# joshuacwnewton/swiftwatcher

Hardware: AMD Instinct MI355X
Metric: frames/sec (segment+classify) on 1080p ROI batches (higher is better)
Workload: dtype f64 (image_filtering), f32 (CNN)

## Files before the change

### swiftwatcher_amd/csrc/cnn_common.h

```cpp
#pragma once
#include "swk_internal.h"

#include <cstring>

namespace swk {

typedef float f16v __attribute__((ext_vector_type(16)));
typedef __bf16 bf16x8 __attribute__((ext_vector_type(8)));

struct Place {
    float *dst;
    int dH, dW, dC, off_y, off_x, c_off;
};
struct Crop {
    int sh, sw, crop_y, crop_x;
};

inline bool place_ok(const Place &p, int h, int w, int c, bool quads, const Crop *crop = nullptr)
{
    if (!p.dst || c < 1 || p.off_y < 0 || p.off_x < 0 || p.off_y + h > p.dH || p.off_x + w > p.dW || p.c_off < 0 || p.c_off + c > p.dC) return false;
    if (quads && ((c & 3) || (p.dC & 3) || (p.c_off & 3) || ((uintptr_t)p.dst & 15))) return false;
    return !crop || (crop->crop_y >= 0 && crop->crop_x >= 0 && crop->crop_y + h <= crop->sh && crop->crop_x + w <= crop->sw);
}

int launch_expand1x1_split_bf16(hipStream_t s, const float *src, int64_t rows, const Crop &cr, int cin, int h, int w, const float *wgt,
                                const float *bias, int cout, const Place &pl);
extern int g_expand_split_bf16;

__device__ __forceinline__ void store_bias_relu(float *q, const f16v &acc, int g, const float4 b)
{
    float4 v;
    v.x = fmaxf(acc[4 * g] + b.x, 0.0f);
    v.y = fmaxf(acc[4 * g + 1] + b.y, 0.0f);
    v.z = fmaxf(acc[4 * g + 2] + b.z, 0.0f);
    v.w = fmaxf(acc[4 * g + 3] + b.w, 0.0f);
    *(float4 *)q = v;
}

__device__ __forceinline__ void split3(float x, __bf16 &a, __bf16 &b, __bf16 &c)
{
    a = (__bf16)x;
    const float r = x - (float)a;
    b = (__bf16)r;
    c = (__bf16)(r - (float)b);
}
inline void split3_host(float x, uint16_t part[3])
{
    for (int i = 0; i < 3; ++i) {
        uint32_t u;
        float back;
        memcpy(&u, &x, 4);
        u = (u + 0x7fffu + ((u >> 16) & 1u)) & 0xffff0000u;
        memcpy(&back, &u, 4);
        part[i] = (uint16_t)(u >> 16);
        x -= back;
    }
}

inline void winograd_U(const float g[9], double U[4][4])
{
    static const double G[4][3] = {{1.0, 0.0, 0.0}, {0.5, 0.5, 0.5}, {0.5, -0.5, 0.5}, {0.0, 0.0, 1.0}};
    double tmp[4][3];
    for (int a = 0; a < 4; ++a)
        for (int c = 0; c < 3; ++c) tmp[a][c] = G[a][0] * g[c] + G[a][1] * g[3 + c] + G[a][2] * g[6 + c];
    for (int a = 0; a < 4; ++a)
        for (int c = 0; c < 4; ++c) U[a][c] = tmp[a][0] * G[c][0] + tmp[a][1] * G[c][1] + tmp[a][2] * G[c][2];
}

template <int N>
__device__ __forceinline__ void lds_dma_copy(unsigned lds, const void *g, unsigned voff)
{
    static_assert(N >= 1 && N <= 3, "1 KB pieces per statement");
    unsigned keep;
#define SWK_LDS_DMA(pieces)                                                                                                 \
    asm volatile("s_mov_b32 %0, m0\n\ts_mov_b32 m0, %2\n\ts_nop 0\n\t" pieces "s_mov_b32 m0, %0" : "=&s"(keep) : "v"(voff), "s"(lds), "s"(g) : "memory")
#define SWK_LDS_DMA_PIECE(offset) "global_load_lds_dwordx4 %1, %3" offset "\n\t"
    if constexpr (N == 1) SWK_LDS_DMA(SWK_LDS_DMA_PIECE(""));
    else if constexpr (N == 2) SWK_LDS_DMA(SWK_LDS_DMA_PIECE("") SWK_LDS_DMA_PIECE(" offset:1024"));
    else SWK_LDS_DMA(SWK_LDS_DMA_PIECE("") SWK_LDS_DMA_PIECE(" offset:1024") SWK_LDS_DMA_PIECE(" offset:2048"));
#undef SWK_LDS_DMA_PIECE
#undef SWK_LDS_DMA
}
template <int KEEP>
__device__ __forceinline__ void lds_dma_wait()
{
    asm volatile("s_waitcnt vmcnt(%0)" ::"n"(KEEP) : "memory");
}

}
```

### swiftwatcher_amd/csrc/cnn_conv1x1.hip

```cpp
#include "cnn_common.h"

namespace swk {

template <int NBLK, int KC, int D, int CS, int NWV>
__global__ __launch_bounds__(64 * NWV) void k_conv1x1_relu_place(const float *__restrict__ src, int64_t rows, int sh, int sw, int cin, int crop_y,
                                                            int crop_x, int h, int w, const float *__restrict__ wgt, const float *__restrict__ bias,
                                                            int cout, float *__restrict__ dst, int dH, int dW, int dC, int off_y, int off_x, int c_off,
                                                            FastDiv fhw, FastDiv fw)
{
    constexpr int NP = 32 * NBLK, PITCH = NP + 1, KH = KC / 2, NV = KH / 4, NB = NBLK / CS, NT = 64 * NWV, SLOTS = NWV / CS;
    static_assert(NBLK % CS == 0 && NWV % CS == 0, "column splits");
    extern __shared__ float lds[];
    const int tid = threadIdx.x, lane = tid & 63, wave = tid >> 6, r = lane & 31, hh = lane >> 5;
    float *lbias = lds + ((cin * PITCH + 3) & ~3);
    const int hw = h * w;
    const int cs = wave % CS;
    const int64_t ntiles = (rows + 31) >> 5, stride = (int64_t)gridDim.x * SLOTS;
    int64_t tile = (int64_t)blockIdx.x * SLOTS + wave / CS;

    auto locate = [&](int64_t t, int64_t &ro) -> const float * {
        const unsigned m = (unsigned)t * 32u + (unsigned)r;
        const bool valid = m < (unsigned)rows;
        const unsigned mm = valid ? m : (unsigned)rows - 1u;
        const unsigned b = fhw.div(mm), rem = mm - b * (unsigned)hw;
        const unsigned y = fw.div(rem), x = rem - y * (unsigned)w;
        ro = valid ? (((int64_t)b * dH + off_y + y) * dW + off_x + x) * (int64_t)dC + c_off + 32 * NB * cs : -1;
        return src + (((int64_t)b * sh + crop_y + y) * sw + crop_x + x) * (int64_t)cin + KH * hh;
    };
    float4 a[D][NV];
    int64_t ro = -1, ro_next = -1;
    const float *p = src, *pn = src;
    if (tile < ntiles) {
        p = locate(tile, ro);
#pragma unroll
        for (int d = 0; d < D; ++d)
#pragma unroll
            for (int v = 0; v < NV; ++v) a[d][v] = *(const float4 *)(p + KC * d + 4 * v);
    }
    for (int co = tid >> 4; co < NP; co += NT / 16)
        for (int c4 = (tid & 15) * 4; c4 < cin; c4 += 64) {
            const float4 wv = co < cout ? *(const float4 *)(wgt + (int64_t)co * cin + c4) : make_float4(0.0f, 0.0f, 0.0f, 0.0f);
            float *q = lds + c4 * PITCH + co;
            q[0] = wv.x; q[PITCH] = wv.y; q[2 * PITCH] = wv.z; q[3 * PITCH] = wv.w;
        }
    for (int i = tid; i < NP; i += NT) lbias[i] = i < cout ? bias[i] : 0.0f;
    __syncthreads();

    for (; tile < ntiles; tile += stride) {
        const bool more = tile + stride < ntiles;
        if (more) pn = locate(tile + stride, ro_next);
        f16v acc[NB];
#pragma unroll
        for (int nb = 0; nb < NB; ++nb)
#pragma unroll
            for (int e = 0; e < 16; ++e) acc[nb][e] = 0.0f;
        for (int kb = 0; kb < cin; kb += KC * D) {
#pragma unroll
            for (int d = 0; d < D; ++d) {
                const int k0 = kb + KC * d;
                float av[KH];
#pragma unroll
                for (int v = 0; v < NV; ++v) { av[4 * v] = a[d][v].x; av[4 * v + 1] = a[d][v].y; av[4 * v + 2] = a[d][v].z; av[4 * v + 3] = a[d][v].w; }
                const int kn = k0 + KC * D;
                if (kn < cin) {
#pragma unroll
                    for (int v = 0; v < NV; ++v) a[d][v] = *(const float4 *)(p + kn + 4 * v);
                } else if (more) {
#pragma unroll
                    for (int v = 0; v < NV; ++v) a[d][v] = *(const float4 *)(pn + kn - cin + 4 * v);
                }
                const float *wrow = lds + (k0 + KH * hh) * PITCH + 32 * NB * cs + r;
                float bw[2][NB];
#pragma unroll
                for (int nb = 0; nb < NB; ++nb) bw[0][nb] = wrow[32 * nb];
#pragma unroll
                for (int i = 0; i < KH; ++i) {
                    if (i < KH - 1) {
#pragma unroll
                        for (int nb = 0; nb < NB; ++nb) bw[(i + 1) & 1][nb] = wrow[(i + 1) * PITCH + 32 * nb];
                    }
#pragma unroll
                    for (int nb = 0; nb < NB; ++nb) acc[nb] = __builtin_amdgcn_mfma_f32_32x32x2f32(bw[i & 1][nb], av[i], acc[nb], 0, 0, 0);
                    if (i < KH - 1) __builtin_amdgcn_sched_group_barrier(0x100 , NB, 0);
                    __builtin_amdgcn_sched_group_barrier(0x008 , NB, 0);
                }
            }
        }
        if (ro >= 0) {
            float *o = dst + ro + 4 * hh;
#pragma unroll
            for (int nb = 0; nb < NB; ++nb)
#pragma unroll
                for (int g = 0; g < 4; ++g) {
                    const int c = nb * 32 + 8 * g;
                    if (32 * NB * cs + c + 4 * hh < cout) store_bias_relu(o + c, acc[nb], g, *(const float4 *)(lbias + 32 * NB * cs + c + 4 * hh));
                }
        }
        p = pn;
        ro = ro_next;
    }
}

template <int NBLK, int KC, int D, int CS, int NWV>
static int launch_conv1x1_d(hipStream_t s, const float *src, int64_t rows, const Crop &cr, int cin, int h, int w, const float *wgt,
                            const float *bias, int cout, const Place &pl)
{
    const size_t lds = (size_t)(((cin * (32 * NBLK + 1) + 3) & ~3) + 32 * NBLK) * sizeof(float);
    static unsigned long long attr_mask = 0;
    if (!ensure_dyn_lds((const void *)k_conv1x1_relu_place<NBLK, KC, D, CS, NWV>, 160 * 1024 - 256, attr_mask)) return SWK_ERR_HIP;
    if (lds > 160 * 1024 - 256 || rows > (int64_t)0x7fffff00) return SWK_ERR_CAPACITY;
    constexpr int SLOTS = NWV / CS;
    const int64_t ntiles = (rows + 31) / 32;
    int64_t blocks = (ntiles + SLOTS - 1) / SLOTS;
    const int64_t by_lds = (int64_t)((160 * 1024 - 256) / lds), by_waves = 16 / NWV;
    const int64_t per_cu = by_lds < 1 ? 1 : (by_lds < by_waves ? by_lds : by_waves);
    const int64_t cap = 256 * per_cu;
    if (blocks > cap) blocks = cap;
    hipLaunchKernelGGL((k_conv1x1_relu_place<NBLK, KC, D, CS, NWV>), dim3((unsigned)blocks), dim3(64 * NWV), lds, s, src, rows, cr.sh, cr.sw, cin,
                       cr.crop_y, cr.crop_x, h, w, wgt, bias, cout, pl.dst, pl.dH, pl.dW, pl.dC, pl.off_y, pl.off_x, pl.c_off, FastDiv((unsigned)(h * w)), FastDiv((unsigned)w));
    return hipGetLastError() == hipSuccess ? SWK_OK : SWK_ERR_HIP;
}

int g_expand_split_bf16 = getenv("SWK_EXPAND_SPLIT_BF16") ? atoi(getenv("SWK_EXPAND_SPLIT_BF16")) : 0;
int g_conv1x1_ring = 0;

#define SWK_C1_ARGS s, src, rows, cr, cin, h, w, wgt, bias, cout, pl
template <int NBLK>
static int launch_conv1x1(hipStream_t s, const float *src, int64_t rows, const Crop &cr, int cin, int h, int w, const float *wgt, const float *bias,
                          int cout, const Place &pl)
{
    constexpr int CS = NBLK >= 6 ? 2 : 1;
    if (g_conv1x1_ring == 0) {
        const int64_t ntiles = (rows + 31) / 32;
        const int nwv = ntiles >= 16 * 160 / CS ? 16 : ntiles >= 8 * 160 / CS ? 8 : 4;
#define SWK_C1_BY_WAVES(KC)                                                              \
        do {                                                                             \
            if (nwv == 16) return launch_conv1x1_d<NBLK, KC, 1, CS, 16>(SWK_C1_ARGS);    \
            if (nwv == 8) return launch_conv1x1_d<NBLK, KC, 1, CS, 8>(SWK_C1_ARGS);      \
            return launch_conv1x1_d<NBLK, KC, 1, CS, 4>(SWK_C1_ARGS);                    \
        } while (0)
        if (cin % 32 == 0) SWK_C1_BY_WAVES(32);
        if (cin == 48) SWK_C1_BY_WAVES(48);
        SWK_C1_BY_WAVES(16);
#undef SWK_C1_BY_WAVES
    }
    if (cin % 32 == 0) {
        const int n = cin / 32, dmax = NBLK >= 6 ? 2 : 4;
        const int d = dmax >= 4 && n % 4 == 0 ? 4 : dmax >= 3 && n % 3 == 0 ? 3 : dmax >= 2 && n % 2 == 0 ? 2 : 1;
        switch (d) {
        case 4: if constexpr (NBLK < 6) return launch_conv1x1_d<NBLK, 32, 4, 1, 8>(SWK_C1_ARGS);
        case 3: if constexpr (NBLK < 6) return launch_conv1x1_d<NBLK, 32, 3, 1, 8>(SWK_C1_ARGS);
        case 2: return launch_conv1x1_d<NBLK, 32, 2, 1, 8>(SWK_C1_ARGS);
        default: return launch_conv1x1_d<NBLK, 32, 1, 1, 8>(SWK_C1_ARGS);
        }
    }
    if (cin == 48) return launch_conv1x1_d<NBLK, 48, 1, 1, 8>(SWK_C1_ARGS);
    return launch_conv1x1_d<NBLK, 16, 1, 1, 8>(SWK_C1_ARGS);
}
#undef SWK_C1_ARGS

}

#pragma GCC visibility push(default)
extern "C" {

int32_t swk_nhwc_conv1x1_bias_relu_place(void *stream, const float *src, int32_t n, int32_t sh, int32_t sw, int32_t cin, int32_t crop_y,
                                         int32_t crop_x, int32_t h, int32_t w, const float *weight, const float *bias, int32_t cout,
                                         float *dst, int32_t dH, int32_t dW, int32_t dC, int32_t off_y, int32_t off_x, int32_t c_off)
{
    const swk::Place pl{dst, dH, dW, dC, off_y, off_x, c_off};
    const swk::Crop cr{sh, sw, crop_y, crop_x};
    if (!src || !weight || !bias || n < 1 || h < 1 || w < 1 || cin < 16 || (cin & 15) || cin > 1024 || cout > 256 ||
        !swk::place_ok(pl, h, w, cout, true, &cr) || ((((uintptr_t)src) | ((uintptr_t)weight)) & 15))
        return SWK_ERR_ARG;
    using namespace swk;
    const int64_t rows = (int64_t)n * h * w;
    hipStream_t s = (hipStream_t)stream;
    if (g_expand_split_bf16 && cout == 4 * cin) {
        const int rc = launch_expand1x1_split_bf16(s, src, rows, cr, cin, h, w, weight, bias, cout, pl);
        if (rc != SWK_ERR_ARG) return rc;
    }
    switch ((cout + 31) / 32) {
    case 1: return launch_conv1x1<1>(s, src, rows, cr, cin, h, w, weight, bias, cout, pl);
    case 2: return launch_conv1x1<2>(s, src, rows, cr, cin, h, w, weight, bias, cout, pl);
    case 3: return launch_conv1x1<3>(s, src, rows, cr, cin, h, w, weight, bias, cout, pl);
    case 4: return launch_conv1x1<4>(s, src, rows, cr, cin, h, w, weight, bias, cout, pl);
    case 6: return launch_conv1x1<6>(s, src, rows, cr, cin, h, w, weight, bias, cout, pl);
    case 8: return launch_conv1x1<8>(s, src, rows, cr, cin, h, w, weight, bias, cout, pl);
    default: return SWK_ERR_ARG;
    }
}

int32_t swk_set_cnn_tuning(int32_t knob, int32_t value)
{
    if (knob == 0 && (value == 0 || value == 1)) { swk::g_conv1x1_ring = value; return SWK_OK; }
    if (knob == 1 && (value == 0 || value == 1)) { swk::g_expand_split_bf16 = value; return SWK_OK; }
    return SWK_ERR_ARG;
}

}
#pragma GCC visibility pop
```

### swiftwatcher_amd/csrc/cnn_wino3x3_bf16s.hip

```cpp
#include "cnn_common.h"

namespace swk {

static int wino_bf16s_spp(int cin, int cout) { return cin == 64 && cout == 256 ? 2 : cin / 16; }

template <int KG> struct WinoVPad { static constexpr int value = KG == 6 ? 3 : 16 / KG; };

template <int NBLK, int SPP>
__global__ __launch_bounds__(64 * NBLK, 2) void k_wino3x3_bf16s_relu_place(const float *__restrict__ src, int nseg, int t, int T,
                                                                          const uint16_t *__restrict__ wu, const float *__restrict__ bias,
                                                                          int cout, float *__restrict__ dst, int dH, int dW, int dC, int off_y,
                                                                          int off_x, int c_off, FastDiv fTT, FastDiv fT)
{
    constexpr int NW = NBLK, NT = 64 * NW, KG = NBLK, CIN = 8 * KG, S = CIN / 16, PHS = S / SPP, SLOTS = 64, NP = 32 * NBLK;
    constexpr int VT = SLOTS + WinoVPad<KG>::value;
    constexpr int WPB = SPP * 3 * 1024;
    static_assert(S % SPP == 0 && NT == SLOTS * KG, "one staging item per thread");
    extern __shared__ uint4 lds_w[];
    char *const Wl = (char *)lds_w;
    uint4 *const V0 = (uint4 *)(Wl + 2 * NW * WPB), *const V1 = V0 + 3 * KG * VT;
    float *const lbias = (float *)(V1 + 3 * KG * VT);
    const int tid = threadIdx.x, lane = tid & 63, wave = tid >> 6, r = lane & 31, hh = lane >> 5;
    const int o = t - 2, TT = T * T;
    const int64_t ntiles = (int64_t)nseg * TT, src_floats = (int64_t)nseg * t * t * CIN;
    const int64_t ntasks = (ntiles + SLOTS - 1) / SLOTS;
    for (int i = tid; i < NP; i += NT) lbias[i] = i < cout ? bias[i] : 0.0f;

    const int sg = tid % KG, sslot = tid / KG;
    unsigned sbase;
    int slim;
    const char *const srcb = (const char *)src;
    auto stage_setup = [&](int64_t task) {
        int64_t m = task * SLOTS + sslot;
        if (m >= ntiles) m = ntiles - 1;
        const unsigned bu = fTT.div((unsigned)m), rem = (unsigned)m - bu * (unsigned)TT, ty = fT.div(rem), tx = rem - ty * (unsigned)T;
        const int64_t b = bu;
        const int64_t base = (((b * t + 2 * ty) * t + 2 * tx) * (int64_t)CIN + 8 * sg) * 4;
        const int64_t lim = src_floats * 4 - 32 - base;
        sbase = (unsigned)base;
        slim = (int)(lim < (1 << 30) ? lim : (1 << 30));
    };
    float4 st[4][2];
    auto stage_issue = [&](int p) {
        const int xi = p >> 2, nu = p & 3;
        const int ra0 = (0x1210 >> (4 * xi)) & 15, ra1 = (0x3122 >> (4 * xi)) & 15;
        const int rb0 = (0x1210 >> (4 * nu)) & 15, rb1 = (0x3122 >> (4 * nu)) & 15;
        const int os[4] = {(ra0 * t + rb0) * (CIN * 4), (ra0 * t + rb1) * (CIN * 4), (ra1 * t + rb0) * (CIN * 4), (ra1 * t + rb1) * (CIN * 4)};
#pragma unroll
        for (int i = 0; i < 4; ++i) {
            const char *q = srcb + (sbase + (unsigned)(os[i] < slim ? os[i] : slim));
            st[i][0] = *(const float4 *)q;
            st[i][1] = *(const float4 *)(q + 16);
        }
    };
    auto stage_store = [&](int p, uint4 *Vn) {
        const float sx = (p >> 2) == 1 ? 1.0f : -1.0f, sn = (p & 3) == 1 ? 1.0f : -1.0f;
        bf16x8 v1, v2, v3;
#pragma unroll
        for (int h = 0; h < 2; ++h) {
            const float a[4] = {st[0][h].x, st[0][h].y, st[0][h].z, st[0][h].w}, b[4] = {st[1][h].x, st[1][h].y, st[1][h].z, st[1][h].w},
                        c[4] = {st[2][h].x, st[2][h].y, st[2][h].z, st[2][h].w}, d[4] = {st[3][h].x, st[3][h].y, st[3][h].z, st[3][h].w};
#pragma unroll
            for (int e = 0; e < 4; ++e) {
                const float v = __builtin_fmaf(__builtin_fmaf(d[e], sn, c[e]), sx, __builtin_fmaf(b[e], sn, a[e]));
                __bf16 x1, x2, x3;
                split3(v, x1, x2, x3);
                v1[4 * h + e] = x1; v2[4 * h + e] = x2; v3[4 * h + e] = x3;
            }
        }
        uint4 *q = Vn + sg * VT + sslot;
        q[0] = __builtin_bit_cast(uint4, v1);
        q[KG * VT] = __builtin_bit_cast(uint4, v2);
        q[2 * KG * VT] = __builtin_bit_cast(uint4, v3);
    };

    const unsigned wvoff = (unsigned)(lane * 16);
    auto w_issue = [&](int g, int buf) {
        const char *gp = (const char *)wu + ((int64_t)g * NW + __builtin_amdgcn_readfirstlane(wave)) * WPB;
        const unsigned l = __builtin_amdgcn_readfirstlane((unsigned)(uintptr_t)(Wl + (buf * NW + wave) * WPB));
#pragma unroll
        for (int sub = 0; sub < SPP; ++sub) lds_dma_copy<3>(l + sub * 3072u, gp + sub * 3072, wvoff);
    };

    int64_t task = blockIdx.x;
    if (task < ntasks) {
        stage_setup(task);
        stage_issue(0);
        stage_store(0, V0);
        w_issue(0, 0);
    }
    lds_dma_wait<0>();
    __syncthreads();
    for (; task < ntasks; task += gridDim.x) {
        int64_t ro[2];
        bool valid[2], vy1[2], vx1[2];
#pragma unroll
        for (int tg = 0; tg < 2; ++tg) {
            const int64_t m = task * SLOTS + tg * 32 + r;
            valid[tg] = m < ntiles;
            const int64_t mm = valid[tg] ? m : ntiles - 1;
            const unsigned bu = fTT.div((unsigned)mm), rem = (unsigned)mm - bu * (unsigned)TT;
            const int ty = (int)fT.div(rem), tx = (int)(rem - (unsigned)ty * (unsigned)T);
            const int64_t b = bu;
            ro[tg] = ((b * dH + off_y + 2 * ty) * dW + off_x + 2 * tx) * (int64_t)dC + c_off + 32 * wave + 4 * hh;
            vy1[tg] = 2 * ty + 1 < o;
            vx1[tg] = 2 * tx + 1 < o;
        }
        const bool more = task + gridDim.x < ntasks;
        f16v Y[2][2][2];
#pragma unroll
        for (int i = 0; i < 2; ++i)
#pragma unroll
            for (int j = 0; j < 2; ++j)
#pragma unroll
                for (int tg = 0; tg < 2; ++tg)
#pragma unroll
                    for (int e = 0; e < 16; ++e) Y[i][j][tg][e] = 0.0f;
        auto phase = [&](const char *Wb, const uint4 *Vc, int s0, f16v *M) {
            const uint4 *wq = (const uint4 *)Wb + lane;
#pragma unroll
            for (int sub = 0; sub < SPP; ++sub) {
                const int s = s0 + sub;
                const bf16x8 u1 = __builtin_bit_cast(bf16x8, wq[(3 * sub) * 64]), u2 = __builtin_bit_cast(bf16x8, wq[(3 * sub + 1) * 64]),
                             u3 = __builtin_bit_cast(bf16x8, wq[(3 * sub + 2) * 64]);
#pragma unroll
                for (int tg = 0; tg < 2; ++tg) {
                    const uint4 *vq = Vc + (2 * s + hh) * VT + 32 * tg + r;
                    const bf16x8 x1 = __builtin_bit_cast(bf16x8, vq[0]), x2 = __builtin_bit_cast(bf16x8, vq[KG * VT]),
                                 x3 = __builtin_bit_cast(bf16x8, vq[2 * KG * VT]);
                    M[tg] = __builtin_amdgcn_mfma_f32_32x32x16_bf16(u1, x3, M[tg], 0, 0, 0);
                    M[tg] = __builtin_amdgcn_mfma_f32_32x32x16_bf16(u2, x2, M[tg], 0, 0, 0);
                    M[tg] = __builtin_amdgcn_mfma_f32_32x32x16_bf16(u3, x1, M[tg], 0, 0, 0);
                    M[tg] = __builtin_amdgcn_mfma_f32_32x32x16_bf16(u1, x2, M[tg], 0, 0, 0);
                    M[tg] = __builtin_amdgcn_mfma_f32_32x32x16_bf16(u2, x1, M[tg], 0, 0, 0);
                    M[tg] = __builtin_amdgcn_mfma_f32_32x32x16_bf16(u1, x1, M[tg], 0, 0, 0);
                }
            }
        };
        for (int p = 0; p < 16; ++p) {
            const uint4 *Vc = (p & 1) ? V1 : V0;
            uint4 *Vn = (p & 1) ? V0 : V1;
            const int pn = (p + 1) & 15;
            if (p == 15 && more) stage_setup(task + gridDim.x);
            const int xi = p >> 2, nu = p & 3;
            const float ax[2] = {xi < 3 ? 1.0f : 0.0f, xi == 0 ? 0.0f : xi == 1 ? 1.0f : -1.0f};
            const float an[2] = {nu < 3 ? 1.0f : 0.0f, nu == 0 ? 0.0f : nu == 1 ? 1.0f : -1.0f};
            f16v M[2];
#pragma unroll
            for (int tg = 0; tg < 2; ++tg)
#pragma unroll
                for (int e = 0; e < 16; ++e) M[tg][e] = 0.0f;
#pragma unroll
            for (int h = 0; h < PHS; ++h) {
                const int g = p * PHS + h, gn = g + 1 == 16 * PHS ? 0 : g + 1;
                w_issue(gn, (g + 1) & 1);
                if (h == 0) stage_issue(pn);
                phase(Wl + ((g & 1) * NW + wave) * WPB, Vc, h * SPP, M);
                if (h == PHS - 1) {
                    stage_store(pn, Vn);
#pragma unroll
                    for (int i = 0; i < 2; ++i)
#pragma unroll
                        for (int j = 0; j < 2; ++j) {
                            const float c = ax[i] * an[j];
                            if (c != 0.0f) {
#pragma unroll
                                for (int tg = 0; tg < 2; ++tg)
#pragma unroll
                                    for (int e = 0; e < 16; ++e) Y[i][j][tg][e] = __builtin_fmaf(M[tg][e], c, Y[i][j][tg][e]);
                            }
                        }
                }
                if (h == 0 && PHS > 1) lds_dma_wait<8>();
                else lds_dma_wait<0>();
                if (h == PHS - 1) __syncthreads();
            }
        }
#pragma unroll
        for (int tg = 0; tg < 2; ++tg) {
            if (!valid[tg]) continue;
#pragma unroll
            for (int i = 0; i < 2; ++i)
#pragma unroll
                for (int j = 0; j < 2; ++j) {
                    if ((i == 1 && !vy1[tg]) || (j == 1 && !vx1[tg])) continue;
                    float *q = dst + ro[tg] + ((int64_t)i * dW + j) * dC;
#pragma unroll
                    for (int gq = 0; gq < 4; ++gq) {
                        const int c = 32 * wave + 8 * gq + 4 * hh;
                        if (c < cout) store_bias_relu(q + 8 * gq, Y[i][j][tg], gq, *(const float4 *)(lbias + c));
                    }
                }
        }
    }
}

template <int NBLK, int SPP>
static int launch_wino3x3_bf16s(hipStream_t s, const float *src, int n, int t, const uint16_t *wu, const float *bias, int cout, const Place &pl)
{
    constexpr int NW = NBLK, KG = NBLK, CIN = 8 * NBLK, VT = 64 + WinoVPad<KG>::value;
    const size_t lds = (size_t)2 * NW * SPP * 3 * 1024 + (size_t)2 * 3 * KG * VT * 16 + 32 * NBLK * sizeof(float);
    static_assert((size_t)2 * NW * SPP * 3 * 1024 + (size_t)2 * 3 * KG * VT * 16 + 32 * NBLK * 4 <= 160 * 1024 - 256, "LDS of one workgroup");
    static unsigned long long attr_mask = 0;
    if (!ensure_dyn_lds((const void *)k_wino3x3_bf16s_relu_place<NBLK, SPP>, 160 * 1024 - 256, attr_mask)) return SWK_ERR_HIP;
    if ((int64_t)n * t * t * CIN * 4 >= ((int64_t)1 << 32)) return SWK_ERR_CAPACITY;
    const int T = (t - 2 + 1) / 2;
    const int64_t ntiles = (int64_t)n * T * T;
    int64_t blocks = (ntiles + 63) / 64;
    const int64_t by_lds = (int64_t)((160 * 1024 - 256) / lds), by_waves = 8 / NW;
    const int64_t per_cu = by_waves < 1 ? 1 : (by_lds < by_waves ? by_lds : by_waves);
    if (blocks > 256 * per_cu) blocks = 256 * per_cu;
    hipLaunchKernelGGL((k_wino3x3_bf16s_relu_place<NBLK, SPP>), dim3((unsigned)blocks), dim3(64 * NW), lds, s, src, n, t, T, wu, bias, cout, pl.dst,
                       pl.dH, pl.dW, pl.dC, pl.off_y, pl.off_x, pl.c_off, FastDiv((unsigned)(T * T)), FastDiv((unsigned)T));
    return hipGetLastError() == hipSuccess ? SWK_OK : SWK_ERR_HIP;
}

}

#pragma GCC visibility push(default)
extern "C" {

int32_t swk_winograd_f2x2_3x3_weights_bf16s(const float *weight, int32_t cout, int32_t cin, uint16_t *out)
{
    if (!weight || !out || cout < 1 || cin < 16 || (cin & 15)) return SWK_ERR_ARG;
    const int spp = swk::wino_bf16s_spp(cin, cout), S = cin / 16, PHS = S / spp, CG = (cout + 31) / 32;
    if (S % spp) return SWK_ERR_ARG;
    for (int64_t i = 0, e = (int64_t)16 * cin * CG * 32 * 3; i < e; ++i) out[i] = 0;
    for (int co = 0; co < cout; ++co)
        for (int ci = 0; ci < cin; ++ci) {
            double U[4][4];
            swk::winograd_U(weight + ((int64_t)co * cin + ci) * 9, U);
            const int s = ci >> 4, ph = s / spp, sub = s % spp, lane = ((ci >> 3) & 1) * 32 + (co & 31), j = ci & 7, cb = co >> 5;
            for (int p = 0; p < 16; ++p) {
                uint16_t part[3];
                swk::split3_host((float)U[p >> 2][p & 3], part);
                const int64_t blk = (((int64_t)p * PHS + ph) * CG + cb) * spp + sub;
                for (int k = 0; k < 3; ++k) out[((blk * 3 + k) * 64 + lane) * 8 + j] = part[k];
            }
        }
    return SWK_OK;
}

int32_t swk_nhwc_conv3x3_winograd_bf16s_bias_relu_place(void *stream, const float *src, int32_t n, int32_t t, int32_t cin,
                                                        const uint16_t *weight_s, const float *bias, int32_t cout, float *dst, int32_t dH,
                                                        int32_t dW, int32_t dC, int32_t off_y, int32_t off_x, int32_t c_off)
{
    const swk::Place pl{dst, dH, dW, dC, off_y, off_x, c_off};
    if (!src || !weight_s || !bias || n < 1 || t < 3 || !swk::place_ok(pl, t - 2, t - 2, cout, true) || (((uintptr_t)src | (uintptr_t)weight_s) & 15))
        return SWK_ERR_ARG;
    using namespace swk;
    hipStream_t s = (hipStream_t)stream;
    if (cin == 16 && cout == 64) return launch_wino3x3_bf16s<2, 1>(s, src, n, t, weight_s, bias, cout, pl);
    if (cin == 32 && cout == 128) return launch_wino3x3_bf16s<4, 2>(s, src, n, t, weight_s, bias, cout, pl);
    if (cin == 48 && cout == 192) return launch_wino3x3_bf16s<6, 3>(s, src, n, t, weight_s, bias, cout, pl);
    if (cin == 64 && cout == 256) return launch_wino3x3_bf16s<8, 2>(s, src, n, t, weight_s, bias, cout, pl);
    return SWK_ERR_ARG;
}

}
#pragma GCC visibility pop
```

Measured before the change: 41470.

## Add shared-weight Winograd bf16 kernel with multiple wave groups per workgroup

Adds a new Winograd 3x3 bf16-split kernel variant in which several wave groups (WCB) in one workgroup share the same LDS weight buffers. Each group handles its own set of tile slots, and the weight DMA is split across the groups. The variant becomes the default for the cin=48 and cin=64 layers, and a new tuning knob selects the layout. The goal is to reuse each staged weight block over more tiles and reduce weight traffic per tile. In exchange, the workgroups are larger, barriers are shared across more waves, and the occupancy and LDS trade-offs change.

```diff
diff --git a/swiftwatcher_amd/csrc/cnn_common.h b/swiftwatcher_amd/csrc/cnn_common.h
--- a/swiftwatcher_amd/csrc/cnn_common.h
+++ b/swiftwatcher_amd/csrc/cnn_common.h
@@ -26,6 +26,7 @@
 int launch_expand1x1_split_bf16(hipStream_t s, const float *src, int64_t rows, const Crop &cr, int cin, int h, int w, const float *wgt,
                                 const float *bias, int cout, const Place &pl);
 extern int g_expand_split_bf16;
+extern int g_wino_bf16s_layout;
 
 __device__ __forceinline__ void store_bias_relu(float *q, const f16v &acc, int g, const float4 b)
 {
diff --git a/swiftwatcher_amd/csrc/cnn_conv1x1.hip b/swiftwatcher_amd/csrc/cnn_conv1x1.hip
--- a/swiftwatcher_amd/csrc/cnn_conv1x1.hip
+++ b/swiftwatcher_amd/csrc/cnn_conv1x1.hip
@@ -195,6 +195,7 @@
 {
     if (knob == 0 && (value == 0 || value == 1)) { swk::g_conv1x1_ring = value; return SWK_OK; }
     if (knob == 1 && (value == 0 || value == 1)) { swk::g_expand_split_bf16 = value; return SWK_OK; }
+    if (knob == 2 && value >= 0 && value <= 2) { swk::g_wino_bf16s_layout = value; return SWK_OK; }
     return SWK_ERR_ARG;
 }
 
diff --git a/swiftwatcher_amd/csrc/cnn_wino3x3_bf16s.hip b/swiftwatcher_amd/csrc/cnn_wino3x3_bf16s.hip
--- a/swiftwatcher_amd/csrc/cnn_wino3x3_bf16s.hip
+++ b/swiftwatcher_amd/csrc/cnn_wino3x3_bf16s.hip
@@ -1,4 +1,6 @@
 #include "cnn_common.h"
+
+#include <type_traits>
 
 namespace swk {
 
@@ -215,6 +217,247 @@
     return hipGetLastError() == hipSuccess ? SWK_OK : SWK_ERR_HIP;
 }
 
+template <int KG> struct WinoVPadW { static constexpr int value = KG == 4 ? 2 : KG == 6 ? 3 : 1; };
+
+typedef __bf16 bf16x4 __attribute__((ext_vector_type(4)));
+
+template <int NBLK, int SPP, int TGW, int WCB, int WPS>
+__global__ __launch_bounds__(64 * NBLK * WCB, WPS) void k_wino3x3_bf16s_shared_relu_place(const float *__restrict__ src, int nseg, int t, int T,
+                                                                                         const uint16_t *__restrict__ wu,
+                                                                                         const float *__restrict__ bias, int cout,
+                                                                                         float *__restrict__ dst, int dH, int dW, int dC, int off_y,
+                                                                                         int off_x, int c_off, FastDiv fTT, FastDiv fT)
+{
+    constexpr int NW = NBLK * WCB, NT = 64 * NW, KG = NBLK, CIN = 8 * KG, S = CIN / 16, PHS = S / SPP, SLOTS = 32 * TGW * WCB, NP = 32 * NBLK;
+    constexpr bool LATE = WPS == 4;
+    constexpr int NH = TGW;
+    constexpr int VT = SLOTS + WinoVPadW<KG>::value;
+    constexpr int WPB = SPP * 3 * 1024;
+    constexpr int PC = 3 * SPP, PC0 = (PC + WCB - 1) / WCB;
+    static_assert(S % SPP == 0 && NT * NH == 2 * SLOTS * KG && (TGW == 1 || TGW == 2) && (WCB == 1 || WCB == 2), "staging items and waves");
+    extern __shared__ uint4 lds_w[];
+    char *const Wl = (char *)lds_w;
+    uint4 *const V0 = (uint4 *)(Wl + 2 * NBLK * WPB), *const V1 = V0 + 3 * KG * VT;
+    float *const lbias = (float *)(V1 + 3 * KG * VT);
+    const int tid = threadIdx.x, lane = tid & 63, r = lane & 31, hh = lane >> 5;
+    const int wv = __builtin_amdgcn_readfirstlane(tid >> 6), cb = wv % NBLK, wj = wv / NBLK, tg0 = wj * TGW;
+    const int o = t - 2, TT = T * T;
+    const int64_t ntiles = (int64_t)nseg * TT, src_floats = (int64_t)nseg * t * t * CIN;
+    const int64_t ntasks = (ntiles + SLOTS - 1) / SLOTS;
+    for (int i = tid; i < NP; i += NT) lbias[i] = i < cout ? bias[i] : 0.0f;
+
+    const int item = NH == 2 ? tid : tid >> 1, shalf = NH == 2 ? 0 : tid & 1;
+    const int sg = item % KG, sslot = item / KG;
+    unsigned sbase;
+    int slim;
+    const char *const srcb = (const char *)src;
+    auto stage_setup = [&](int64_t task) {
+        int64_t m = task * SLOTS + sslot;
+        if (m >= ntiles) m = ntiles - 1;
+        const unsigned bu = fTT.div((unsigned)m), rem = (unsigned)m - bu * (unsigned)TT, ty = fT.div(rem), tx = rem - ty * (unsigned)T;
+        const int64_t b = bu;
+        const int64_t base = (((b * t + 2 * ty) * t + 2 * tx) * (int64_t)CIN + 8 * sg + 4 * shalf) * 4;
+        const int64_t lim = src_floats * 4 - 16 * NH - base;
+        sbase = (unsigned)base;
+        slim = (int)(lim < (1 << 30) ? lim : (1 << 30));
+    };
+    float4 st[4][NH];
+    auto stage_issue = [&](int p) {
+        const int xi = p >> 2, nu = p & 3;
+        const int ra0 = (0x1210 >> (4 * xi)) & 15, ra1 = (0x3122 >> (4 * xi)) & 15;
+        const int rb0 = (0x1210 >> (4 * nu)) & 15, rb1 = (0x3122 >> (4 * nu)) & 15;
+        const int os[4] = {(ra0 * t + rb0) * (CIN * 4), (ra0 * t + rb1) * (CIN * 4), (ra1 * t + rb0) * (CIN * 4), (ra1 * t + rb1) * (CIN * 4)};
+#pragma unroll
+        for (int i = 0; i < 4; ++i) {
+            const char *q = srcb + (sbase + (unsigned)(os[i] < slim ? os[i] : slim));
+#pragma unroll
+            for (int h = 0; h < NH; ++h) st[i][h] = *(const float4 *)(q + 16 * h);
+        }
+    };
+    auto stage_store = [&](int p, uint4 *Vn) {
+        const float sx = (p >> 2) == 1 ? 1.0f : -1.0f, sn = (p & 3) == 1 ? 1.0f : -1.0f;
+        bf16x4 v1[NH], v2[NH], v3[NH];
+#pragma unroll
+        for (int h = 0; h < NH; ++h) {
+            const float a[4] = {st[0][h].x, st[0][h].y, st[0][h].z, st[0][h].w}, b[4] = {st[1][h].x, st[1][h].y, st[1][h].z, st[1][h].w},
+                        c[4] = {st[2][h].x, st[2][h].y, st[2][h].z, st[2][h].w}, d[4] = {st[3][h].x, st[3][h].y, st[3][h].z, st[3][h].w};
+#pragma unroll
+            for (int e = 0; e < 4; ++e) {
+                const float v = __builtin_fmaf(__builtin_fmaf(d[e], sn, c[e]), sx, __builtin_fmaf(b[e], sn, a[e]));
+                __bf16 x1, x2, x3;
+                split3(v, x1, x2, x3);
+                v1[h][e] = x1; v2[h][e] = x2; v3[h][e] = x3;
+            }
+        }
+        uint4 *q = Vn + sg * VT + sslot;
+        if constexpr (NH == 2) {
+            const uint2 a1 = __builtin_bit_cast(uint2, v1[0]), b1 = __builtin_bit_cast(uint2, v1[NH - 1]), a2 = __builtin_bit_cast(uint2, v2[0]),
+                        b2 = __builtin_bit_cast(uint2, v2[NH - 1]), a3 = __builtin_bit_cast(uint2, v3[0]), b3 = __builtin_bit_cast(uint2, v3[NH - 1]);
+            q[0] = make_uint4(a1.x, a1.y, b1.x, b1.y);
+            q[KG * VT] = make_uint4(a2.x, a2.y, b2.x, b2.y);
+            q[2 * KG * VT] = make_uint4(a3.x, a3.y, b3.x, b3.y);
+        } else {
+            ((uint2 *)q)[shalf] = __builtin_bit_cast(uint2, v1[0]);
+            ((uint2 *)(q + KG * VT))[shalf] = __builtin_bit_cast(uint2, v2[0]);
+            ((uint2 *)(q + 2 * KG * VT))[shalf] = __builtin_bit_cast(uint2, v3[0]);
+        }
+    };
+
+    const unsigned wvoff = (unsigned)(lane * 16);
+    auto w_pieces = [&](auto first, auto count, unsigned l, const char *gp) {
+        constexpr int F = decltype(first)::value, N = decltype(count)::value;
+#pragma unroll
+        for (int i = 0; i + 3 <= N; i += 3) lds_dma_copy<3>(l + (F + i) * 1024u, gp + (F + i) * 1024, wvoff);
+        if constexpr (N % 3 != 0) lds_dma_copy<N % 3>(l + (F + N - N % 3) * 1024u, gp + (F + N - N % 3) * 1024, wvoff);
+    };
+    auto w_issue = [&](int g, int buf) {
+        const char *gp = (const char *)wu + ((int64_t)g * NBLK + cb) * WPB;
+        const unsigned l = __builtin_amdgcn_readfirstlane((unsigned)(uintptr_t)(Wl + (buf * NBLK + cb) * WPB));
+        if (WCB == 1 || wj == 0) w_pieces(std::integral_constant<int, 0>(), std::integral_constant<int, PC0>(), l, gp);
+        else w_pieces(std::integral_constant<int, PC0>(), std::integral_constant<int, PC - PC0>(), l, gp);
+    };
+
+    int64_t task = blockIdx.x;
+    if (task < ntasks) {
+        stage_setup(task);
+        stage_issue(0);
+        stage_store(0, V0);
+        w_issue(0, 0);
+    }
+    lds_dma_wait<0>();
+    __syncthreads();
+    for (; task < ntasks; task += gridDim.x) {
+        const bool more = task + gridDim.x < ntasks;
+        f16v Y[2][2][TGW];
+#pragma unroll
+        for (int i = 0; i < 2; ++i)
+#pragma unroll
+            for (int j = 0; j < 2; ++j)
+#pragma unroll
+                for (int tg = 0; tg < TGW; ++tg)
+#pragma unroll
+                    for (int e = 0; e < 16; ++e) Y[i][j][tg][e] = 0.0f;
+        auto phase = [&](const char *Wb, const uint4 *Vc, int s0, f16v *M) {
+            const uint4 *wq = (const uint4 *)Wb + lane;
+#pragma unroll
+            for (int sub = 0; sub < SPP; ++sub) {
+                const int s = s0 + sub;
+                const bf16x8 u1 = __builtin_bit_cast(bf16x8, wq[(3 * sub) * 64]), u2 = __builtin_bit_cast(bf16x8, wq[(3 * sub + 1) * 64]),
+                             u3 = __builtin_bit_cast(bf16x8, wq[(3 * sub + 2) * 64]);
+#pragma unroll
+                for (int tg = 0; tg < TGW; ++tg) {
+                    const uint4 *vq = Vc + (2 * s + hh) * VT + 32 * (tg0 + tg) + r;
+                    const bf16x8 x1 = __builtin_bit_cast(bf16x8, vq[0]), x2 = __builtin_bit_cast(bf16x8, vq[KG * VT]),
+                                 x3 = __builtin_bit_cast(bf16x8, vq[2 * KG * VT]);
+                    M[tg] = __builtin_amdgcn_mfma_f32_32x32x16_bf16(u1, x3, M[tg], 0, 0, 0);
+                    M[tg] = __builtin_amdgcn_mfma_f32_32x32x16_bf16(u2, x2, M[tg], 0, 0, 0);
+                    M[tg] = __builtin_amdgcn_mfma_f32_32x32x16_bf16(u3, x1, M[tg], 0, 0, 0);
+                    M[tg] = __builtin_amdgcn_mfma_f32_32x32x16_bf16(u1, x2, M[tg], 0, 0, 0);
+                    M[tg] = __builtin_amdgcn_mfma_f32_32x32x16_bf16(u2, x1, M[tg], 0, 0, 0);
+                    M[tg] = __builtin_amdgcn_mfma_f32_32x32x16_bf16(u1, x1, M[tg], 0, 0, 0);
+                }
+                if constexpr (WPS == 4) __builtin_amdgcn_sched_barrier(0);
+            }
+        };
+        for (int p = 0; p < 16; ++p) {
+            const uint4 *Vc = (p & 1) ? V1 : V0;
+            uint4 *Vn = (p & 1) ? V0 : V1;
+            const int pn = (p + 1) & 15;
+            if (p == 15 && more) stage_setup(task + gridDim.x);
+            const int xi = p >> 2, nu = p & 3;
+            const float ax[2] = {xi < 3 ? 1.0f : 0.0f, xi == 0 ? 0.0f : xi == 1 ? 1.0f : -1.0f};
+            const float an[2] = {nu < 3 ? 1.0f : 0.0f, nu == 0 ? 0.0f : nu == 1 ? 1.0f : -1.0f};
+            f16v M[TGW];
+#pragma unroll
+            for (int tg = 0; tg < TGW; ++tg)
+#pragma unroll
+                for (int e = 0; e < 16; ++e) M[tg][e] = 0.0f;
+#pragma unroll
+            for (int h = 0; h < PHS; ++h) {
+                const int g = p * PHS + h, gn = g + 1 == 16 * PHS ? 0 : g + 1;
+                w_issue(gn, (g + 1) & 1);
+                if (h == 0 && !LATE) stage_issue(pn);
+                phase(Wl + ((g & 1) * NBLK + cb) * WPB, Vc, h * SPP, M);
+                if (h == PHS - 1) {
+                    if (LATE) stage_issue(pn);
+                    stage_store(pn, Vn);
+#pragma unroll
+                    for (int i = 0; i < 2; ++i)
+#pragma unroll
+                        for (int j = 0; j < 2; ++j) {
+                            const float c = ax[i] * an[j];
+                            if (c != 0.0f) {
+#pragma unroll
+                                for (int tg = 0; tg < TGW; ++tg)
+#pragma unroll
+                                    for (int e = 0; e < 16; ++e) Y[i][j][tg][e] = __builtin_fmaf(M[tg][e], c, Y[i][j][tg][e]);
+                            }
+                        }
+                }
+                if (h == 0 && PHS > 1) lds_dma_wait<LATE ? 0 : 4 * NH>();
+                else lds_dma_wait<0>();
+                if (h == PHS - 1 || WCB > 1) __syncthreads();
+            }
+        }
+        int le = lane;
+        asm volatile("" : "+v"(le));
+        const int re = le & 31, he = le >> 5;
+        int64_t ro[TGW];
+        bool valid[TGW], vy1[TGW], vx1[TGW];
+#pragma unroll
+        for (int tg = 0; tg < TGW; ++tg) {
+            const int64_t m = task * SLOTS + (tg0 + tg) * 32 + re;
+            valid[tg] = m < ntiles;
+            const int64_t mm = valid[tg] ? m : ntiles - 1;
+            const unsigned bu = fTT.div((unsigned)mm), rem = (unsigned)mm - bu * (unsigned)TT;
+            const int ty = (int)fT.div(rem), tx = (int)(rem - (unsigned)ty * (unsigned)T);
+            const int64_t b = bu;
+            ro[tg] = ((b * dH + off_y + 2 * ty) * dW + off_x + 2 * tx) * (int64_t)dC + c_off + 32 * cb + 4 * he;
+            vy1[tg] = 2 * ty + 1 < o;
+            vx1[tg] = 2 * tx + 1 < o;
+        }
+#pragma unroll
+        for (int tg = 0; tg < TGW; ++tg) {
+            if (!valid[tg]) continue;
+#pragma unroll
+            for (int i = 0; i < 2; ++i)
+#pragma unroll
+                for (int j = 0; j < 2; ++j) {
+                    if ((i == 1 && !vy1[tg]) || (j == 1 && !vx1[tg])) continue;
+                    float *q = dst + ro[tg] + ((int64_t)i * dW + j) * dC;
+#pragma unroll
+                    for (int gq = 0; gq < 4; ++gq) {
+                        const int c = 32 * cb + 8 * gq + 4 * he;
+                        if (c < cout) store_bias_relu(q + 8 * gq, Y[i][j][tg], gq, *(const float4 *)(lbias + c));
+                    }
+                }
+        }
+    }
+}
+
+template <int NBLK, int SPP, int TGW, int WCB, int WPS>
+static int launch_wino3x3_bf16s_shared(hipStream_t s, const float *src, int n, int t, const uint16_t *wu, const float *bias, int cout,
+                                       const Place &pl)
+{
+    constexpr int KG = NBLK, CIN = 8 * NBLK, SLOTS = 32 * TGW * WCB, VT = SLOTS + WinoVPadW<KG>::value;
+    constexpr size_t lds = (size_t)2 * NBLK * SPP * 3 * 1024 + (size_t)2 * 3 * KG * VT * 16 + 32 * NBLK * sizeof(float);
+    constexpr int per_cu = 4 * WPS / (NBLK * WCB);
+    static_assert(per_cu >= 1 && per_cu * lds <= 160 * 1024 - 256, "LDS of a CU's workgroups");
+    static unsigned long long attr_mask = 0;
+    if (!ensure_dyn_lds((const void *)k_wino3x3_bf16s_shared_relu_place<NBLK, SPP, TGW, WCB, WPS>, 160 * 1024 - 256, attr_mask)) return SWK_ERR_HIP;
+    if ((int64_t)n * t * t * CIN * 4 >= ((int64_t)1 << 32)) return SWK_ERR_CAPACITY;
+    const int T = (t - 2 + 1) / 2;
+    const int64_t ntiles = (int64_t)n * T * T;
+    int64_t blocks = (ntiles + SLOTS - 1) / SLOTS;
+    if (blocks > 256 * per_cu) blocks = 256 * per_cu;
+    hipLaunchKernelGGL((k_wino3x3_bf16s_shared_relu_place<NBLK, SPP, TGW, WCB, WPS>), dim3((unsigned)blocks), dim3(64 * NBLK * WCB), lds, s, src, n, t,
+                       T, wu, bias, cout, pl.dst, pl.dH, pl.dW, pl.dC, pl.off_y, pl.off_x, pl.c_off, FastDiv((unsigned)(T * T)),
+                       FastDiv((unsigned)T));
+    return hipGetLastError() == hipSuccess ? SWK_OK : SWK_ERR_HIP;
+}
+
+int g_wino_bf16s_layout = 0;
+
 }
 
 #pragma GCC visibility push(default)
@@ -250,10 +493,23 @@
         return SWK_ERR_ARG;
     using namespace swk;
     hipStream_t s = (hipStream_t)stream;
+    const int knob = g_wino_bf16s_layout;
     if (cin == 16 && cout == 64) return launch_wino3x3_bf16s<2, 1>(s, src, n, t, weight_s, bias, cout, pl);
-    if (cin == 32 && cout == 128) return launch_wino3x3_bf16s<4, 2>(s, src, n, t, weight_s, bias, cout, pl);
-    if (cin == 48 && cout == 192) return launch_wino3x3_bf16s<6, 3>(s, src, n, t, weight_s, bias, cout, pl);
-    if (cin == 64 && cout == 256) return launch_wino3x3_bf16s<8, 2>(s, src, n, t, weight_s, bias, cout, pl);
+    if (cin == 32 && cout == 128) {
+        const int lay = knob ? knob : 1;
+        if (lay == 2) return launch_wino3x3_bf16s_shared<4, 2, 2, 2, 2>(s, src, n, t, weight_s, bias, cout, pl);
+        return launch_wino3x3_bf16s<4, 2>(s, src, n, t, weight_s, bias, cout, pl);
+    }
+    if (cin == 48 && cout == 192) {
+        const int lay = knob ? knob : 2;
+        if (lay == 2) return launch_wino3x3_bf16s_shared<6, 3, 1, 2, 3>(s, src, n, t, weight_s, bias, cout, pl);
+        return launch_wino3x3_bf16s<6, 3>(s, src, n, t, weight_s, bias, cout, pl);
+    }
+    if (cin == 64 && cout == 256) {
+        const int lay = knob ? knob : 2;
+        if (lay == 2) return launch_wino3x3_bf16s_shared<8, 2, 1, 2, 4>(s, src, n, t, weight_s, bias, cout, pl);
+        return launch_wino3x3_bf16s<8, 2>(s, src, n, t, weight_s, bias, cout, pl);
+    }
     return SWK_ERR_ARG;
 }
 
```

Result: faster. 42190 (median of 6 runs) (+1.7%).
